# bmorris3/gadfly

Measured on AMD Instinct MI355X. Metric: GP log-likelihood evals/sec (N=1e6, J=30), higher is better.
Workload: dtype f64

## Files before the change

### gadfly_amd/_lib.py

```python
import ctypes
import os
import subprocess

_HERE = os.path.dirname(os.path.abspath(__file__))
CSRC = os.path.join(_HERE, "csrc")
SO_PATH = os.path.join(CSRC, "libgadfly_hip.so")
if os.environ.get("GADFLY_SO"):
    SO_PATH = os.path.abspath(os.environ["GADFLY_SO"])
SOURCES = [os.path.join(CSRC, "gadfly_hip.hip"), os.path.join(CSRC, "gadfly_stored.hip"),
           os.path.join(CSRC, "gadfly_linear.hip"), os.path.join(CSRC, "gadfly_series.hip"),
           os.path.join(CSRC, "gadfly_dense.hip"),
           os.path.join(CSRC, "gadfly_ls.hip"), os.path.join(CSRC, "gadfly_grad.hip"),
           os.path.join(CSRC, "gadfly_solve.hip"), os.path.join(CSRC, "gadfly_predict.hip"),
           os.path.join(CSRC, "gadfly_var.hip"), os.path.join(CSRC, "gadfly_spectral.hip"),
           os.path.join(CSRC, "gadfly_fisher.hip"), os.path.join(CSRC, "gadfly_rhs.hip"),
           os.path.join(CSRC, "gadfly_lsfft.hip"), os.path.join(CSRC, "gadfly_gradtp.hip"),
           os.path.join(CSRC, "gadfly_detrend.hip"), os.path.join(CSRC, "gadfly_linmodel.hip"),
           os.path.join(CSRC, "gadfly_quadform.hip"), os.path.join(CSRC, "gadfly_gradw.hip")]
HEADER = os.path.join(os.path.dirname(_HERE), "include", "gadfly_hip.h")

GF_SOLVE_LOWER, GF_SOLVE_UPPER, GF_MATMUL_LOWER = 0, 1, 2
GF_SWEEP_AUTO, GF_SWEEP_COLUMN, GF_SWEEP_TILED = 0, 1, 2
GF_SWEEP_ZERO_START = 0x100
GF_SWEEP_LONG_SPAN = 0x200
GF_SWEEP_AXIS_PROVEN = 0x400
GF_MAX_WIDTH = 256
GF_GRAD_MAX_WIDTH = 63
GF_GRAD_WORKSPACE_BYTES = 16 << 30
GF_SOLVE_MAX_WIDTH = 63
GF_SOLVE_WORKSPACE_BYTES = 16 << 30
GF_DETREND_MAX_ORDER = 8
GF_LINEAR_MAX_COLS = 255

_lib = None

_vp = ctypes.c_void_p
_i64 = ctypes.c_int64
_int = ctypes.c_int
_dbl = ctypes.c_double

SIGNATURES = {
    "gf_version": (_int, []),
    "gf_last_error": (ctypes.c_char_p, []),
    "gf_leading_dim": (_int, [_int]),
    "gf_build_matrices": (_int, [_int, _i64, _i64, _int, _int, _int] + [_vp] * 7
                          + [_vp, _i64, _vp, _i64] + [_vp] * 4 + [_vp]),
    "gf_state_size": (_i64, [_int]),
    "gf_state_cols": (_int, [_int]),
    "gf_factor": (_int, [_int, _i64, _i64, _int, _int] + [_vp] * 4 + [_vp, _i64]
                  + [_vp] * 6 + [_vp]),
    "gf_scaled_supported": (_int, [_int]),
    "gf_scaled_span": (_dbl, [_int]),
    "gf_scaled_wide_supported": (_int, [_int]),
    "gf_build_scaled": (_int, [_int, _i64, _i64, _int, _int, _int] + [_vp] * 8 + [_int]
                        + [_vp, _i64, _vp, _i64] + [_vp] * 4 + [_vp]),
    "gf_factor_scaled": (_int, [_int, _i64, _i64, _int, _int] + [_vp] * 5 + [_vp, _i64]
                         + [_vp] * 5 + [_vp]),
    "gf_fused_supported": (_int, [_int, _int]),
    "gf_fused_state_size": (_i64, [_int, _int]),
    "gf_loglike_fused": (_int, [_int, _i64, _i64, _int, _int, _int, _int, _int] + [_vp] * 8
                         + [_vp, _i64, _vp, _i64, _vp, _i64] + [_vp] * 5 + [_vp]),
    "gf_steady_size": (_i64, []),
    "gf_loglike_steady": (_int, [_int, _i64, _i64, _int, _int, _int, _int, _int] + [_vp] * 8
                          + [_vp, _i64, _vp, _i64, _vp, _i64] + [_vp] * 5 + [_vp, _i64] + [_vp]),
    "gf_steady_sweep": (_int, [_int, _i64, _i64, _int, _int, _int, _int, _int] + [_vp] * 8
                        + [_vp, _i64, _vp, _i64, _vp, _i64] + [_vp] * 5 + [_vp, _i64] + [_vp]),
    "gf_reduce_tile_steady": (_int, [_int, _i64, _i64] + [_vp] * 5 + [_int, _vp]),
    "gf_steady_sweep_reduced": (_int, [_int, _i64, _i64, _int, _int, _int, _int, _int] + [_vp] * 8
                                + [_vp, _i64, _vp, _i64, _vp, _i64] + [_vp] * 5 + [_vp, _i64, _vp, _int] + [_vp]),
    "gf_steady_sweep_rank1": (_int, [_int, _i64, _i64, _int, _int, _int, _int, _int] + [_vp] * 8
                              + [_vp, _i64, _vp, _i64, _vp, _i64] + [_vp] * 5 + [_vp, _i64, _vp, _int, _vp] + [_vp]),
    "gf_steady_finish": (_int, [_int, _i64, _int, _int, _int, _int] + [_vp] * 5 + [_vp, _i64, _vp, _i64]
                         + [_vp] * 3 + [_vp]),
    "gf_steady_finish_window": (_int, [_int, _i64, _int, _int, _int, _int] + [_vp] * 5 + [_vp, _i64, _vp, _i64]
                                + [_vp] * 3 + [_i64, _i64] + [_vp]),
    "gf_steady_chunk_size": (_i64, [_i64, _int]),
    "gf_steady_finish_chunked": (_int, [_int, _i64, _int, _int, _int, _int] + [_vp] * 5 + [_vp, _i64, _vp, _i64]
                                 + [_vp] * 3 + [_i64, _i64, _int, _vp] + [_vp]),
    "gf_sample_fused": (_int, [_int, _i64, _i64, _int, _int, _int, _int, _int] + [_vp] * 8
                        + [_vp, _i64, _vp, _i64, _vp, _i64] + [_vp] * 5 + [_vp]),
    "gf_chunk_sweep": (_int, [_int, _i64, _i64, _int, _int, _int, _int, _int, _int, _int, _int] + [_vp] * 8
                       + [_vp, _i64, _vp, _i64, _vp, _i64] + [_vp] * 9 + [_vp]),
    "gf_fused_row_stride": (_int, [_int, _int]),
    "gf_scaled_propagator": (_int, [_int, _i64, _int, _int, _vp, _vp, _vp, _vp]),
    "gf_chunk_linear": (_int, [_int, _int, _i64, _i64, _int, _int, _int, _int, _int]
                        + [_vp] * 8 + [_vp]),
    "gf_chunk_linear_combine": (_int, [_int, _int, _i64, _i64, _int, _int, _int] + [_vp] * 5
                                + [_vp]),
    "gf_dense_solve": (_int, [_int, _int, _int] + [_vp] * 2 + [_vp]),
    "gf_dense_solve_logdet": (_int, [_int, _int, _int] + [_vp] * 3 + [_vp]),
    "gf_dense_width": (_int, [_int]),
    "gf_wide_combine_work": (_i64, [_int, _int, _int]),
    "gf_wide_combine": (_int, [_int, _i64, _i64, _int, _int] + [_vp] * 7 + [_vp]),
    "gf_chunk_corrections_work": (_i64, [_int, _int]),
    "gf_chunk_corrections": (_int, [_int, _int, _int, _int, _int] + [_vp] * 6 + [_vp]),
    "gf_wide_gram": (_int, [_int, _i64, _i64, _int, _int, _int, _int, _int] + [_vp] * 5 + [_vp]),
    "gf_lft_tree_work": (_i64, [_int, _int, _int]),
    "gf_lft_tree_scan": (_int, [_int, _int, _int] + [_vp] * 8 + [_vp]),
    "gf_bgemm": (_int, [_int, _int, _int, _int, _int, _int, _vp, _int, _i64, _vp, _int, _i64,
                        _vp, _int, _i64, _vp, _int, _i64, _vp]),
    "gf_chunk_segment_transitions": (_int, [_int, _int, _int] + [_vp] * 4 + [_vp]),
    "gf_chunk_linear_combine_seg": (_int, [_int, _int, _int, _int, _int] + [_vp] * 6 + [_vp]),
    "gf_chunk_transition": (_int, [_int, _i64, _i64, _int, _int, _int, _int, _int, _int] + [_vp] * 9 + [_vp]),
    "gf_chunk_transition_wide": (_int, [_int, _i64, _i64, _int, _int, _int, _int] + [_vp] * 7 + [_vp]),
    "gf_chunk_combine": (_int, [_int, _int, _int] + [_vp] * 5 + [_vp]),
    "gf_chunk_combine_tree_work": (_i64, [_int, _int, _int]),
    "gf_chunk_combine_tree": (_int, [_int, _int, _int, _int] + [_vp] * 8 + [_vp]),
    "gf_reduce_work": (_i64, [_i64]),
    "gf_reduce_tile": (_int, [_int, _i64] + [_vp] * 4 + [_int, _vp]),
    "gf_loglike_finish": (_int, [_int, _i64] + [_vp] * 4 + [_vp]),
    "gf_solve": (_int, [_int, _int, _i64, _int, _int, _int] + [_vp] * 6 + [_vp]),
    "gf_solve_chunk": (_int, [_int, _int, _i64, _i64, _int, _int, _int] + [_vp] * 7 + [_int, _vp]),
    "gf_solve_chunk_rhs": (_int, [_int, _int, _i64, _i64, _int, _int, _int, _int] + [_vp] * 7 + [_int, _vp]),
    "gf_chunk_diag_scan": (_int, [_int, _int, _int, _int, _vp, _vp, _vp]),
    "gf_cross_covariance": (_int, [_int, _i64, _int, _int, _int] + [_vp] * 6 + [_vp, _i64, _vp, _i64, _vp, _vp]),
    "gf_interp_work": (_i64, [_i64]),
    "gf_interp_plan": (_int, [_i64, _vp, _vp, _dbl, _vp, _vp, _vp]),
    "gf_interp_fill": (_int, [_i64, _vp, _vp, _vp, _dbl, _vp, _vp, _vp, _vp]),
    "gf_psd_power": (_int, [_int, _i64, _i64, _dbl, _vp, _vp, _vp]),
    "gf_psd_bin": (_int, [_int, _i64, _int, _vp, _vp, _vp, _dbl, _vp, _vp, _vp]),
    "gf_ls_segments": (_int, [_i64]),
    "gf_ls_work": (_i64, [_i64, _i64, _int]),
    "gf_ls_power": (_int, [_int, _i64, _i64, _i64, _int, _int] + [_vp] * 8 + [_vp]),
    "gf_lsfft_grid": (_i64, [_i64]),
# ... 168 lines not shown
```

### gadfly_amd/csrc/gadfly_hip.hip

```cpp

#include <hip/hip_runtime.h>
#include <atomic>
#include <utility>
#include <type_traits>
#include <stdint.h>
#include <stdio.h>
#include <stdarg.h>
#include <math.h>

#include "../../include/gadfly_hip.h"
#include "gf_internal.h"

#define FM_INLINE __device__ __forceinline__
#include "fastmath.h"
#include "gf_wave.h"
#include "gf_sweep.h"

template <unsigned long long BITS>
__device__ __forceinline__ double fm_local_constant(const int z) {
    return __hiloint2double((int)(unsigned)(BITS >> 32) ^ z, (int)(unsigned)(BITS & 0xffffffffull) ^ z);
}
#define GF_K(x) fm_local_constant<__builtin_bit_cast(unsigned long long, (double)(x))>(fm_z)
__device__ __forceinline__ double fm_exp_local(const double x) {
    int fm_z;
// ... 1231 lines not shown
        for (int j = 0; j < 16; ++j) a[j] = 0.0;
#pragma unroll 4
        for (int k = 0; k < 64; ++k) {
            const double m = s_m[i][k];
#pragma unroll
            for (int j = 0; j < 16; ++j) a[j] = fma(m, s_m[k][c0 + j], a[j]);
        }
    }
#pragma unroll
    for (int j = 0; j < 16; ++j) P[64 * i + c0 + j] = a[j];
}

__global__ void __launch_bounds__(64)
k_steady_chunk_sum(const int B, const int64_t N, const int32_t *__restrict__ info, const double *__restrict__ steady_,
                   const int64_t sw_lo, const int64_t sw_hi, const int64_t chunk_rows,
                   const double *__restrict__ ws_, const int64_t ws_ld, double *__restrict__ acc_) {
    const int pr = blockIdx.x * 64 + threadIdx.x;
    if (pr >= B) return;
    const int64_t sw = steady_chunk_problem(pr, N, info, steady_, sw_lo, sw_hi, chunk_rows, 1);
    if (sw == 0) return;
    const int nch = (int)((N - sw + chunk_rows - 1) / chunk_rows);
    const double *__restrict__ slot = ws_ + (size_t)pr * ws_ld + CH_P;
    double q = 0.0;
    for (int c = 0; c < nch; ++c) q += slot[c * CH_SLOT + 64];
    const double dinf = steady_[(size_t)pr * ST_SIZE + ST_D];
    double *__restrict__ a = acc_ + (size_t)pr * RED_NACC;
    a[0] += (double)(N - sw) * log(dinf);
    a[1] += q / dinf;
    a[2] = fmin(a[2], dinf);
}

constexpr int R1_RR = 0, R1_RI = 64, R1_YR = 128, R1_YI = 192, R1_XR = 256, R1_XI = 320;
constexpr int R1_D = 384, R1_SG = 385;

__device__ __forceinline__ void half_wave_sums(double v, double &lo, double &up) {
    v += dpp_get<0xB1, 0xf>(v);
    v += dpp_get<0x4E, 0xf>(v);
    v += dpp_get<0x141, 0xf>(v);
    v += dpp_get<0x140, 0xf>(v);
    v += dpp_get<0x142, 0xf>(v);
    lo = read_lane(v, 31);
    up = read_lane(v, 63);
}

__device__ __forceinline__ double lane_select(const unsigned long long lanes, const double v, const double keep) {
    int lo = __double2loint(keep), hi = __double2hiint(keep);
    asm("v_cndmask_b32 %0, %0, %1, %2" : "+v"(lo) : "v"(__double2loint(v)), "s"(lanes));
    asm("v_cndmask_b32 %0, %0, %1, %2" : "+v"(hi) : "v"(__double2hiint(v)), "s"(lanes));
    return __hiloint2double(hi, lo);
}

constexpr int R1_UNROLL = 8;

__global__ void __launch_bounds__(64, 2)
k_steady_rank1(const int64_t N, const int64_t n_first, const int Jc, const double gap,
               const double *__restrict__ ac_, const double *__restrict__ bc_,
               const double *__restrict__ cc_, const double *__restrict__ dc_,
               const double *__restrict__ diag_add_, const double *__restrict__ cmax_,
               const double *__restrict__ t_, const int64_t t_bs,
               const double *__restrict__ diag_, const int64_t diag_bs,
               const double *__restrict__ y_, const int64_t y_bs,
               double *__restrict__ d_, double *__restrict__ z_, double *__restrict__ S_state,
               int32_t *__restrict__ info, double *__restrict__ steady_, const int64_t arm_from,
               const double *__restrict__ dt_, double *acc_, const int acc_init) {
    const int lane = threadIdx.x, pr = blockIdx.x;
    const int h = lane >> 5, c = lane & 31;
    int64_t tile_lim = 0;
#define R1_EXIT(lim) do { if (acc_) { tile_lim = (lim); goto tile_sums; } return; } while (0)
  {
    if (info[pr] != 0) R1_EXIT(steady_rows_stored(steady_, pr, N, n_first));
    double *__restrict__ hdr = steady_ + (size_t)pr * ST_SIZE;
    if (hdr[ST_SW] > 0.0) R1_EXIT(steady_rows_stored(steady_, pr, N, n_first));
    const double *__restrict__ tg = t_ + (size_t)pr * t_bs + n_first;
    const double *__restrict__ yg = y_ + (size_t)pr * y_bs + n_first;
    double *__restrict__ dg = d_ + (size_t)pr * N;
    double *__restrict__ zg = z_ + (size_t)pr * N;
    double *__restrict__ Sg = S_state + (size_t)pr * (64 * 64);
    const bool term = c < Jc, fl = lane == 63;
    const size_t ck = (size_t)pr * Jc + (term ? c : 0);
    const double ck_c = term ? cc_[ck] : 0.0, ck_d = term ? dc_[ck] : 0.0;
    const double ck_a = term ? ac_[ck] : 0.0, ck_b = term ? bc_[ck] : 0.0;
    const double wmax = wave_max(fmax(ck_c, fabs(ck_d)));
    const double gthr = gap / cmax_[pr], jthr = 2e-6 / wmax;
    const double delta = dt_[pr];
    double lr, li;
    {
        double sn, cs;
        fm_sincos(ck_d * delta, &sn, &cs);
        const double e = fm_exp(-ck_c * delta);
        lr = e * cs;
        li = -e * sn;
    }
    double rr, ri, Yr, Yi, Xr, Xi, d, sg;
    if (n_first == 0) {
        d = (diag_ ? diag_[(size_t)pr * diag_bs] : 0.0) + diag_add_[pr];
        sg = fast_rcp(d);
        rr = term ? 1.0 : 0.0;
        ri = 0.0;
        Yr = term ? lr : 0.0;
        Yi = term ? li : 0.0;
        Xr = h ? Yr : 0.0;
        Xi = h ? Yi : 0.0;
    } else {
        rr = Sg[R1_RR + lane]; ri = Sg[R1_RI + lane];
        Yr = Sg[R1_YR + lane]; Yi = Sg[R1_YI + lane];
        Xr = Sg[R1_XR + lane]; Xi = Sg[R1_XI + lane];
        d = Sg[R1_D]; sg = Sg[R1_SG];
    }
    constexpr double thr = ST_THR;
    int cnt = __builtin_amdgcn_readfirstlane((int)hdr[ST_CNT]);
    int fill = __builtin_amdgcn_readfirstlane((int)hdr[ST_FILL]);
    int32_t fail = 0;
    double inv = fast_rcp(d);
    double kr = rr * inv, ki = ri * inv;
    const int64_t last = N - 1;
    auto row_of = [&](const int64_t cb) { const int64_t i = cb + lane; return i < last ? i : last; };
    double t_nx, tp_nx, y_nx;
    {
        const int64_t i = row_of(0);
        t_nx = tg[i];
        tp_nx = (n_first + i > 0) ? tg[i - 1] : t_nx - delta;
        y_nx = yg[i];
    }
    double sd = 0.0, sz = 0.0, sr, si, beta, yv_blk = 0.0;
    auto row_front = [&](const int j) __attribute__((always_inline)) {
        const double yy = read_lane(yv_blk, j);
        double sf;
        half_wave_sums(fma(ck_a, Xr, -(ck_b * Xi)), sf, beta);
        const double zn = yy - sf;
// ... 39 lines not shown
        return bad ? (int)__ffsll((long long)bad) - 1 : -1;
    };
    auto flush = [&](const int64_t nb, const int rows) __attribute__((always_inline)) {
        if (lane < rows) { dg[nb + lane] = sd; zg[nb + lane] = sz; }
    };
    const int g0lo = (int)(n_first & (ST_GRID - 1));
    const int ja = (ST_GRID - g0lo) & (ST_GRID - 1);
    __builtin_amdgcn_s_setprio(GF_CHAIN_PRIO);
    for (int64_t nb = 0; nb < N; nb += 64) {
        const int lim = (int)(N - nb < 64 ? N - nb : 64);
        yv_blk = y_nx;
        asm volatile("" : "+v"(yv_blk));
        {
            const double dt = t_nx - tp_nx;
            const bool bad = (dt > gthr) || !(fabs(dt - delta) < jthr);
            if (__any(bad) && lane == 0) hdr[ST_VIOL] = 1.0;
            const int64_t i = row_of(nb + 64);
            t_nx = tg[i];
            tp_nx = (n_first + i > 0) ? tg[i - 1] : t_nx - delta;
            y_nx = yg[i];
        }
        int jf;
        if (ja < lim) {
            plain_rows(0, ja);
            row_front(ja);
            jf = first_failed(ja + 1);
            if (jf < 0) {
                const int64_t n = nb + ja, gn = n_first + n;
                if (gn >= arm_from) {
                    const double x = fl ? d : (h ? ki : kr);
                    double *__restrict__ slot = hdr + ST_RING + (size_t)((gn / ST_GRID) & (ST_LAG - 1)) * 64 + lane;
                    const double xo = *slot;
                    *slot = x;
                    const double dx = fl ? 0.0 : fabs(x - xo);
                    const double mdx = wave_max(dx), mx = wave_max(fl ? 0.0 : fabs(x));
                    const double dold = read_lane(xo, 63);
                    const bool ok = fill >= ST_LAG && mdx <= thr * mx && fabs(d - dold) <= thr * d;
                    cnt = ok ? cnt + 1 : 0;
                    fill = fill < ST_LAG ? fill + 1 : fill;
                    if (lane == 0) { hdr[ST_CNT] = (double)cnt; hdr[ST_FILL] = (double)fill; }
                    if (cnt >= ST_COUNT && gn >= ST_DLAG) {
                        if (h == 0) {
                            hdr[ST_GR + c] = kr;
                            hdr[ST_GI + c] = ki;
                            hdr[ST_SR + c] = sr;
                            hdr[ST_SI + c] = si;
                        }
                        if (lane == 0) {
                            hdr[ST_SW] = (double)(gn + 1);
                            hdr[ST_D] = d;
                            hdr[ST_DT] = (tg[n] - tg[n - ST_DLAG]) * (1.0 / ST_DLAG);
                        }
                        flush(nb, ja + 1);
                        R1_EXIT(n + 1);
                    }
                }
                row_back();
                plain_rows(ja + 1, lim);
                jf = first_failed(lim);
            }
        } else {
            plain_rows(0, lim);
            jf = first_failed(lim);
        }
        if (jf >= 0) {
            flush(nb, jf);
            const int64_t gf = n_first + nb + jf + 1;
            fail = (int32_t)(gf > 0x7fffffff ? 0x7fffffff : gf);
            break;
        }
        flush(nb, lim);
    }
    if (fail) {
        if (lane == 0) info[pr] = fail;
        R1_EXIT(N);
    }
    Sg[R1_RR + lane] = rr; Sg[R1_RI + lane] = ri;
    Sg[R1_YR + lane] = Yr; Sg[R1_YI + lane] = Yi;
    Sg[R1_XR + lane] = Xr; Sg[R1_XI + lane] = Xi;
    if (lane == 0) { Sg[R1_D] = d; Sg[R1_SG] = sg; }
    R1_EXIT(N);
  }
#undef R1_EXIT
tile_sums:
    __builtin_amdgcn_s_setprio(0);
    __builtin_amdgcn_fence(__ATOMIC_RELEASE, "workgroup");
    __builtin_amdgcn_fence(__ATOMIC_ACQUIRE, "workgroup");
    steady_tile_sums(d_ + (size_t)pr * N, z_ + (size_t)pr * N, N, tile_lim, acc_ + (size_t)pr * RED_NACC, acc_init, lane);
}

struct PhiRing {
    static constexpr int PD = 8;
    static constexpr int USL = 72, RSL = 64;
    static constexpr int OD = 64, OE = 66, OZ = 68;
    double u[PD][USL];
    double r[PD + 1][RSL];
};

struct PhiCursor {
    uintptr_t cu, cr, mask;
    unsigned long long ustep;
    bool in_u, in_r;
    unsigned lds_u, lds_r;
    template <int rows = 64>
    __device__ __forceinline__ void init(PhiRing &R, const int lane, const size_t pb, const double *ut_,
                                         const double *rbar_, const double *dbar_, const double *de_,
                                         const double *zbar_) {
        cu = reinterpret_cast<uintptr_t>(ut_ + pb * 64 + 2 * (lane & 31));
        cr = reinterpret_cast<uintptr_t>(rbar_ + pb * 64 + 2 * (lane & 31));
        mask = ~(uintptr_t)0;
        ustep = 64 * 8;
        if (lane >= 32) {
            const double *sp = (lane == 32) ? dbar_ : (lane == 33) ? de_ : zbar_;
            cu = reinterpret_cast<uintptr_t>(sp + pb);
            mask = ~(uintptr_t)15;
            ustep = 8;
        }
        in_u = lane < (rows + 1) / 2 || (lane >= 32 && lane < 35);
        in_r = lane < (rows + 1) / 2;
        lds_u = __builtin_amdgcn_readfirstlane((unsigned)reinterpret_cast<uintptr_t>(&R.u[0][0]));
        lds_r = __builtin_amdgcn_readfirstlane((unsigned)reinterpret_cast<uintptr_t>(&R.r[0][0]));
    }
    __device__ __forceinline__ void issue(const int64_t m, const int after) {
        const unsigned sl = (unsigned)(m & (PhiRing::PD - 1));
        if (in_u) glds16(reinterpret_cast<const void *>(cu & mask), lds_u + sl * (PhiRing::USL * 8), after);
        if (in_r) glds16(reinterpret_cast<const void *>(cr), lds_r + sl * (PhiRing::RSL * 8), after);
        cu += ustep;
        cr += 64 * 8;
    }
};

template <int NT>
struct PhiGram {
    static constexpr int LD = 80;
    static constexpr int NACC = NT * (NT + 1) / 2;
    double hs[16][LD];
    double sv[16];
};

template <int NT>
__device__ __forceinline__ void phi_gram_flush(PhiGram<NT> &Gm, d4 (&acc)[PhiGram<NT>::NACC], const int lane) {
// ... 1443 lines not shown
                                   info, stream));
}

int64_t gf_steady_size(void) { return ST_SIZE; }

int gf_loglike_steady(int B, int64_t N, int64_t n_first, int Jr, int Jc, int block,
                      int gen_period, int variant,
                      const double *ar, const double *cr, const double *ac,
                      const double *bc, const double *cc, const double *dc,
                      const double *diag_add, const double *cmax,
                      const double *t, int64_t t_bs, const double *diag, int64_t diag_bs,
                      const double *y, int64_t y_bs,
                      double *d, double *z, double *S_state, double *F_state,
                      int32_t *info, double *steady, int64_t arm_from, void *stream) {
    if (!steady) return gf_internal_error(-1, "gf_loglike_steady: null pointer");
    SweepCall c = sweep_call("gf_loglike_steady", B, N, n_first, Jr, Jc, block, gen_period, variant, ar, cr, ac, bc, cc, dc,
                             diag_add, cmax, t, t_bs, diag, diag_bs, y, y_bs, d, z, S_state, F_state, info, stream);
    c.steady = steady; c.arm_from = arm_from;
    return launch_sweep(c);
}

int gf_steady_sweep(int B, int64_t N, int64_t n_first, int Jr, int Jc, int block,
                    int gen_period, int variant,
                    const double *ar, const double *cr, const double *ac,
                    const double *bc, const double *cc, const double *dc,
                    const double *diag_add, const double *cmax,
                    const double *t, int64_t t_bs, const double *diag, int64_t diag_bs,
                    const double *y, int64_t y_bs,
                    double *d, double *z, double *S_state, double *F_state,
                    int32_t *info, double *steady, int64_t arm_from, void *stream) {
    if (!steady) return gf_internal_error(-1, "gf_steady_sweep: null pointer");
    SweepCall c = sweep_call("gf_steady_sweep", B, N, n_first, Jr, Jc, block, gen_period, variant, ar, cr, ac, bc, cc, dc,
                             diag_add, cmax, t, t_bs, diag, diag_bs, y, y_bs, d, z, S_state, F_state, info, stream);
    c.steady = steady; c.arm_from = arm_from; c.tail = false;
    return launch_sweep(c);
}

int gf_steady_sweep_reduced(int B, int64_t N, int64_t n_first, int Jr, int Jc, int block,
                            int gen_period, int variant,
                            const double *ar, const double *cr, const double *ac,
                            const double *bc, const double *cc, const double *dc,
                            const double *diag_add, const double *cmax,
                            const double *t, int64_t t_bs, const double *diag, int64_t diag_bs,
                            const double *y, int64_t y_bs,
                            double *d, double *z, double *S_state, double *F_state,
                            int32_t *info, double *steady, int64_t arm_from, double *acc, int init, void *stream) {
    if (!steady || !acc) return gf_internal_error(-1, "gf_steady_sweep_reduced: null pointer");
    SweepCall c = sweep_call("gf_steady_sweep_reduced", B, N, n_first, Jr, Jc, block, gen_period, variant, ar, cr, ac, bc,
                             cc, dc, diag_add, cmax, t, t_bs, diag, diag_bs, y, y_bs, d, z, S_state, F_state, info, stream);
    c.steady = steady; c.arm_from = arm_from; c.tail = false; c.acc = acc; c.acc_init = init ? 1 : 0;
    return launch_sweep(c);
}

int gf_steady_sweep_rank1(int B, int64_t N, int64_t n_first, int Jr, int Jc, int block,
                          int gen_period, int variant,
                          const double *ar, const double *cr, const double *ac,
                          const double *bc, const double *cc, const double *dc,
                          const double *diag_add, const double *cmax,
                          const double *t, int64_t t_bs, const double *diag, int64_t diag_bs,
                          const double *y, int64_t y_bs,
                          double *d, double *z, double *S_state, double *F_state,
                          int32_t *info, double *steady, int64_t arm_from, double *acc, int init,
                          const double *dt, void *stream) {
    const SweepCall c = sweep_call("gf_steady_sweep_rank1", B, N, n_first, Jr, Jc, block, gen_period, variant, ar, cr, ac,
                                   bc, cc, dc, diag_add, cmax, t, t_bs, diag, diag_bs, y, y_bs, d, z, S_state, F_state,
                                   info, stream);
    const char *who = c.who;
    if (B < 1 || N < 1) return gf_internal_error(-1, "%s: empty problem (N=%lld)", who, (long long)N);
    if (check_block(who, block) || check_n_first(who, n_first, block)) return -1;
    if (!t || !y || !d || !z || !S_state || !info || !diag_add || !cmax || !ac || !bc || !cc || !dc || !steady || !dt)
        return gf_internal_error(-1, "%s: null pointer", who);
    if (check_sweep_options(who, gen_period, variant & ~(GF_SWEEP_ZERO_START | GF_SWEEP_LONG_SPAN), Jr, Jc)) return -1;
    if ((variant & GF_SWEEP_ZERO_START) || !sweep_tiled(variant & ~GF_SWEEP_LONG_SPAN, Jr, Jc) || Jc < 1 || arm_from < 0)
        return gf_internal_error(-1, "%s: steady mode is for the streamed lane-tiled sweep only (Jr = 0, Jc <= 31; Jc=%d)", who, Jc);
    hipLaunchKernelGGL(k_steady_rank1, dim3(c.B), dim3(64), 0, c.st, c.N, c.n_first, c.Jc, sweep_gap(block, variant),
                       c.ac, c.bc, c.cc, c.dc, c.diag_add, c.cmax, c.t, c.t_bs, c.diag, c.diag_bs, c.y, c.y_bs, c.d, c.z,
                       c.S_state, c.info, steady, arm_from, dt, acc, init ? 1 : 0);
    return check_launch(who);
}

static int check_finish(const char *who, int B, int64_t N, int Jr, int Jc, int block) {
    if (B < 1 || N < 1) return gf_internal_error(-1, "%s: empty problem (B=%d, N=%lld)", who, B, (long long)N);
    if (Jr != 0 || Jc < 1 || Jc > 31)
        return gf_internal_error(-1, "%s: steady mode is for the lane-tiled sweep only (Jr = 0, Jc <= 31; Jr=%d, Jc=%d)", who, Jr, Jc);
    return check_block(who, block);
}
static int check_window(const char *who, int64_t sw_lo, int64_t sw_hi) {
    if (sw_lo < 0 || sw_hi < sw_lo)
        return gf_internal_error(-1, "%s: the window of switch rows needs 0 <= sw_lo <= sw_hi (sw_lo=%lld, sw_hi=%lld)", who,
                                 (long long)sw_lo, (long long)sw_hi);
    return 0;
}

static int steady_finish_launch(const char *who, int B, int64_t N, int Jr, int Jc, int block, int variant,
                                const double *ac, const double *bc, const double *cc, const double *dc,
                                const double *cmax, const double *t, int64_t t_bs, const double *y, int64_t y_bs,
                                const int32_t *info, double *steady, double *acc, int64_t sw_lo, int64_t sw_hi,
                                void *stream) {
    if (check_finish(who, B, N, Jr, Jc, block)) return -1;
    if (!ac || !bc || !cc || !dc || !cmax || !t || !y || !info || !steady || !acc)
        return gf_internal_error(-1, "%s: null pointer", who);
    if (check_window(who, sw_lo, sw_hi)) return -1;
    if (sw_lo == sw_hi) return 0;
    const double gap = sweep_gap(block, variant & ~GF_SWEEP_AXIS_PROVEN);
    const bool proven = (variant & GF_SWEEP_AXIS_PROVEN) != 0;
    if (!dispatch_rows((2 * Jc + 3) / 4 * 4, [&](auto r) {
            constexpr int R = decltype(r)::value;
            hipLaunchKernelGGL((proven ? k_steady_finish<R, true> : k_steady_finish<R, false>), dim3(B), dim3(64), 0,
                               (hipStream_t)stream, N, Jc, gap, ac, bc, cc, dc, cmax, t, t_bs, y, y_bs, info, steady, acc,
                               sw_lo, sw_hi);
        }))
        return gf_internal_error(-1, "%s: internal dispatch error", who);
    return check_launch(who);
}

int gf_steady_finish(int B, int64_t N, int Jr, int Jc, int block, int variant,
                     const double *ac, const double *bc, const double *cc, const double *dc, const double *cmax,
                     const double *t, int64_t t_bs, const double *y, int64_t y_bs,
                     const int32_t *info, double *steady, double *acc, void *stream) {
    return steady_finish_launch("gf_steady_finish", B, N, Jr, Jc, block, variant, ac, bc, cc, dc, cmax, t, t_bs, y, y_bs,
                                info, steady, acc, 0, INT64_MAX, stream);
}

int gf_steady_finish_window(int B, int64_t N, int Jr, int Jc, int block, int variant,
                            const double *ac, const double *bc, const double *cc, const double *dc, const double *cmax,
                            const double *t, int64_t t_bs, const double *y, int64_t y_bs,
                            const int32_t *info, double *steady, double *acc,
                            int64_t sw_lo, int64_t sw_hi, void *stream) {
    return steady_finish_launch("gf_steady_finish_window", B, N, Jr, Jc, block, variant, ac, bc, cc, dc, cmax, t, t_bs,
                                y, y_bs, info, steady, acc, sw_lo, sw_hi, stream);
// ... 251 lines not shown
```

### gadfly_amd/engine.py

```python
import contextlib
import functools
import math
import typing

import numpy as np

from . import _lib


def _on_device(method):
    @functools.wraps(method)
    def wrapper(self, *args, **kwargs):
        with self.torch.cuda.device(self.device):
            return method(self, *args, **kwargs)
    return wrapper


@functools.lru_cache(maxsize=None)
def _scaled_span(long_span):
    return float(_lib.load().gf_scaled_span(1 if long_span else 0))


def _coeff_pack(coeffs_list):
    Jr = len(coeffs_list[0][0])
# ... 763 lines not shown
        def padded(x):
            buf = torch.zeros((x.shape[0] * x.shape[1] + 4,), **f64)
            buf[:x.numel()] = x.reshape(-1)
            return buf[:x.numel()].view(x.shape[0], x.shape[1]), buf

        t = rows(t, "t")
        self.N = int(t.shape[1])
        self._tmax = float(t.abs().max()) if axis_stats is None else float(axis_stats[0])
        self.t, self._tpad = padded(t)
        y = rows(y, "y")
        if y.shape[1] != self.N:
            raise ValueError("dimension mismatch")
        self.y, self._ypad = padded(y)
        self.diag = None
        if diag is not None:
            diag = rows(diag, "diag")
            if diag.shape[1] != self.N:
                raise ValueError("dimension mismatch")
            self.diag, self._dpad = padded(diag)
        self._diag_amax = None if self.diag is None else self.diag.amax(dim=1)
        self._coeff_host = (real, comp, diag_add, c)
        self._coeffs_list = list(coeffs_list)
        B, ld = self.B, self.ld
        self.scaled = bool(self.lib.gf_scaled_supported(self.W)) and not force_v1
        self.scaled_wide = bool(self.lib.gf_scaled_wide_supported(self.W)) and not force_v1
        self.allow_fused = bool(allow_fused) and self.scaled and self.W <= 63
        self.allow_wide = (bool(allow_fused) and not force_v1 and self.W > 63
                           and bool(self.lib.gf_fused_supported(self.Jr, self.Jc)))
        self.sweep_variant = _lib.GF_SWEEP_AUTO
        self.generator_period = 4
        self.two_sweep = False
        self.steady_state = True
        self.steady_used = False
        self._steady = None
        self._steady_axis = None
        self._steady_cad_max = None
        self._steady_scanned = None
        self.steady_axis_proven = True
        self._steady_from = 0
        self._steady_skip = 0
        self._steady_feedback = None
        self.finish_events = []
        self.steady_overlap = True
        self._steady_split = 0
        self._steady_mid = 0
        self._steady_chunk_blocks = None
        self._steady_chunk_ws = None
        self._steady_mid_ws = None
        self._finish_side = None
        self._finish_mid_side = None
        self._simds = None
        self.steady_sweep_reduces = True
        self.steady_rank1 = True
        self.rank1_used = False
        self._rank1_dt = None
        self._rank1_cond = None
        T = int(min(max(int(tile_rows), 1), self.N))
        if T < self.N:
            T = max(64, T // 64 * 64)
        self.tile_rows = T
        tt = self.t[0]
        if axis_stats is not None:
            self._dt_med = float(axis_stats[1])
        else:
            self._dt_med = float(torch.median(tt[1:] - tt[:-1])) if self.N > 1 else 0.0
        self.axis_stats = (self._tmax, self._dt_med)
        self._pack = self._make_pack(*self._coeff_host)
        self.generator_period = self.period_for_condition(self.NOMINAL_COND) if self.generator_period > 1 else 1
        self.generator_period = min(self.generator_period, 4)

        def rows_buf():
            return torch.zeros((B * T + 2, ld), **f64)

        self._rows_buf = rows_buf
        self._nbuf = 2 if (T < self.N and overlap_build) else 1
        self.bufs = None
        self.d = torch.empty((B, T), **f64)
        self.z = torch.empty((B, T), **f64)
        nS = 64 * 64 if self.scaled else int(self.lib.gf_state_size(self.W))
        if self.allow_wide:
            nS = max(nS, int(self.lib.gf_fused_state_size(self.Jr, self.Jc)))
        nF = 64 if self.scaled else int(self.lib.gf_state_cols(self.W))
        self.S_state = torch.empty((B, nS), **f64)
        self.F_state = torch.empty((B, nF), **f64)
        self.acc = torch.empty((B, 3), **f64)
        self.work = torch.empty((B * int(self.lib.gf_reduce_work(T)),), **f64)
        self.info = torch.zeros((B,), dtype=torch.int32, device=self.device)
        self.out = torch.empty((B,), **f64)
        self.overlap_build = bool(overlap_build)
        self.side = torch.cuda.Stream(device=self.device) if self.overlap_build else None
        self.time_factor = False
        self.factor_events = []

    _bs = staticmethod(_bs)

    def _alloc_bufs(self):
        torch = self.torch
        f64 = dict(dtype=torch.float64, device=self.device)
        n = self.B * self.tile_rows + 2
        self.bufs = [dict(a=torch.zeros((n,), **f64), U=self._rows_buf(), V=self._rows_buf(),
                          P=None if (self.scaled or self.scaled_wide) else self._rows_buf(),
                          de=torch.zeros((n,), **f64))
                     for _ in range(self._nbuf)]

    def _fused_ok(self):
        return self.allow_fused and self._pack.dmax * self._tmax < SINCOS_RANGE
# ... 185 lines not shown
        T, N, B = self.tile_rows, self.N, self.B
        pack = self._pack
        block, variant = sweep_options(pack, self.sweep_variant)
        per_tile = sweep_head(pack, B, 0, 0, self.Jr, self.Jc, block, int(self.generator_period), variant, self.t,
                              self.diag, self.y, self.d, self.z, self.S_state, self.F_state, self.info)[3:]
        self.kernel_used = "fused-wide" if self.W > 63 else "fused"
        arm_from = self._steady_arm_from()
        start = None if arm_from is None else self._steady_plan(arm_from)
        self.rank1_used = arm_from is not None and self._rank1_ok(arm_from)
        if self.rank1_used:
            start = 0
            if self._rank1_dt is None:
                span = (self.t[:, -1] - self.t[:, 0]) / float(max(N - 1, 1))
                self._rank1_dt = span.expand(B).contiguous()
        self.steady_used = start is not None
        if self.steady_used:
            if self._steady is None:
                self._steady = torch.empty((B, int(lib.gf_steady_size())), dtype=torch.float64, device=self.device)
            self._steady.zero_()
        ntiles = (N + T - 1) // T
        overlap = self.steady_used and self.steady_overlap and B >= self.STEADY_OVERLAP_MIN_B
        split = self._steady_split if overlap else 0
        k_e = split // T - 1 if 0 < split < N else -1
        if not 0 <= k_e < ntiles - 1:
            split, k_e = 0, -1
        mid_end = self._steady_mid if split and B >= self.STEADY_MIDDLE_MIN_B else 0
        k_m = mid_end // T - 1 if mid_end % T == 0 else -1
        if not k_e < k_m < ntiles - 1:
            mid_end, k_m = 0, -1
        windows = steady_windows(split, mid_end)
        used = []
        finish_variant = self._finish_variant(pack, block, variant) if self.steady_used else variant

        def side_stream(middle):
            which = "_finish_mid_side" if middle else "_finish_side"
            if getattr(self, which) is None:
                setattr(self, which, torch.cuda.Stream(device=self.device))
            if getattr(self, which) not in used:
                used.append(getattr(self, which))
            return getattr(self, which)

        def chunked(stream, window, cb, which):
            cb = self._steady_chunk_blocks or cb
            ws = getattr(self, which)
            if ws is None or ws[1] != cb:
                ws = (torch.empty((B, int(lib.gf_steady_chunk_size(N, cb))), dtype=torch.float64, device=self.device), cb)
                setattr(self, which, ws)
            finish("gf_steady_finish_chunked", stream, window[0], window[1], cb, p(ws[0]))

        def finish(name, stream, *tail):
            with _timed(torch, self.time_factor, stream, self.finish_events):
                self._finish_launch(name, stream, pack, block, finish_variant, *tail)

        for k in range(ntiles):
            n0 = k * T
            rows = min(T, N - n0)
            args = (B, rows, n0) + per_tile
            steady_tile = self.steady_used and n0 + rows > start
            reduced = steady_tile and split and k > k_e and self.steady_sweep_reduces
            with _timed(torch, self.time_factor, main, self.factor_events, rows):
                if self.rank1_used:
                    st = lib.gf_steady_sweep_rank1(*args, p(self._steady), 0, p(self.acc) if reduced else None,
                                                   1 if k == 0 else 0, p(self._rank1_dt), main.cuda_stream)
                    _lib.check(st, "gf_steady_sweep_rank1")
                elif reduced:
                    st = lib.gf_steady_sweep_reduced(*args, p(self._steady), arm_from, p(self.acc), 1 if k == 0 else 0,
                                                     main.cuda_stream)
                    _lib.check(st, "gf_steady_sweep_reduced")
                elif steady_tile:
                    st = lib.gf_steady_sweep(*args, p(self._steady), arm_from, main.cuda_stream)
                    _lib.check(st, "gf_steady_sweep")
                else:
                    st = lib.gf_loglike_fused(*args, main.cuda_stream)
                    _lib.check(st, "gf_loglike_fused")
            if reduced:
                pass
            elif steady_tile:
                st = lib.gf_reduce_tile_steady(B, rows, n0, p(self.d), p(self.z), p(self._steady), p(self.work),
                                               p(self.acc), 1 if k == 0 else 0, main.cuda_stream)
                _lib.check(st, "gf_reduce_tile_steady")
            else:
                st = lib.gf_reduce_tile(B, rows, p(self.d), p(self.z), p(self.work), p(self.acc),
                                        1 if k == 0 else 0, main.cuda_stream)
                _lib.check(st, "gf_reduce_tile")
            if k == k_e or k == k_m:
                side = side_stream(k == k_m and self.steady_middle_stream)
                side.wait_event(main.record_event())
                if k == k_e:
                    finish("gf_steady_finish_window", side, *windows[0])
                else:
                    chunked(side, windows[1], steady_chunk_blocks(N, 8), "_steady_mid_ws")
        if self.steady_used:
            if split:
                if mid_end:
                    if self._simds is None:
                        self._simds = 4 * torch.cuda.get_device_properties(self.device).multi_processor_count
                    cb = steady_final_chunk_blocks(N, B, self._simds)
                else:
                    cb = steady_chunk_blocks(N, 8)
                chunked(main, windows[-1], cb, "_steady_chunk_ws")
                for side in used:
                    main.wait_stream(side)
            else:
                finish("gf_steady_finish", main)
            sw = self._steady[:, 0]
            swi = torch.where(sw > 0.0, sw, torch.full_like(sw, float("inf")))
            fb = torch.stack([swi.min(), torch.kthvalue(swi, B - B // 8).values,
                              torch.kthvalue(swi, B - B // 64).values, sw.max(), self._rank1_conditions().max()])
            host = torch.zeros((5,), dtype=torch.float64, pin_memory=True)
            host.copy_(torch.where(torch.isfinite(fb), fb, torch.zeros_like(fb)), non_blocking=True)
            done = torch.cuda.Event()
            done.record(main)
            self._steady_feedback = (host, done)
        out = torch.empty((B,), dtype=torch.float64, device=self.device)
        st = lib.gf_loglike_finish(B, N, p(self.acc), p(self.info), p(out), None,
                                   main.cuda_stream)
        _lib.check(st, "gf_loglike_finish")
        return out

    STEADY_PROBE = 16
    STEADY_OVERLAP_MIN_B = 64
    STEADY_MIDDLE_MIN_B = 512
    steady_middle_stream = True

    def _steady_plan(self, arm_from):
        fb = self._steady_feedback
        if fb is not None and fb[1].query():
            (first, most, mid, latest), self._steady_feedback = (int(v) for v in fb[0][:4]), None
            if len(fb[0]) > 4:
                self._rank1_cond = float(fb[0][4])
            if first > 0:
                self._steady_from = max(0, first - self.STEADY_MIN_ROWS - self.tile_rows)
                self._steady_skip = 0
            else:
                self._steady_from, self._steady_skip = 0, self.STEADY_PROBE - 1
            self._steady_split, self._steady_mid = steady_boundaries(self.N, self.tile_rows, most, mid, latest)
        if self._steady_skip > 0:
            self._steady_skip -= 1
            return None
        return max(arm_from, self._steady_from)

    RANK1_JITTER = 1e-7
    RANK1_COND_LIMIT = 1e5
    RANK1_MIN_ROWS = 32768
# ... 495 lines not shown
```

### include/gadfly_hip.h

```cpp
#ifndef GADFLY_HIP_H
#define GADFLY_HIP_H

#include <stdint.h>

#ifdef __cplusplus
extern "C" {
#endif

#define GF_MAX_WIDTH 256

#define GF_SOLVE_LOWER   0
#define GF_SOLVE_UPPER   1
#define GF_MATMUL_LOWER  2

#define GF_SWEEP_AUTO    0
#define GF_SWEEP_COLUMN  1
#define GF_SWEEP_TILED   2
#define GF_SWEEP_ZERO_START 0x100
#define GF_SWEEP_LONG_SPAN 0x200
#define GF_SWEEP_AXIS_PROVEN 0x400

int gf_version(void);
const char *gf_last_error(void);

// ... 34 lines not shown
int gf_fused_supported(int Jr, int Jc);
int64_t gf_fused_state_size(int Jr, int Jc);
int gf_loglike_fused(int B, int64_t N, int64_t n_first, int Jr, int Jc, int block,
                     int gen_period, int variant,
                     const double *ar, const double *cr, const double *ac,
                     const double *bc, const double *cc, const double *dc,
                     const double *diag_add, const double *cmax,
                     const double *t, int64_t t_bs, const double *diag, int64_t diag_bs,
                     const double *y, int64_t y_bs,
                     double *d, double *z, double *S_state, double *F_state,
                     int32_t *info, void *stream);

int64_t gf_steady_size(void);
int gf_loglike_steady(int B, int64_t N, int64_t n_first, int Jr, int Jc, int block,
                      int gen_period, int variant,
                      const double *ar, const double *cr, const double *ac,
                      const double *bc, const double *cc, const double *dc,
                      const double *diag_add, const double *cmax,
                      const double *t, int64_t t_bs, const double *diag, int64_t diag_bs,
                      const double *y, int64_t y_bs,
                      double *d, double *z, double *S_state, double *F_state,
                      int32_t *info, double *steady, int64_t arm_from, void *stream);

int gf_steady_sweep(int B, int64_t N, int64_t n_first, int Jr, int Jc, int block,
                    int gen_period, int variant,
                    const double *ar, const double *cr, const double *ac,
                    const double *bc, const double *cc, const double *dc,
                    const double *diag_add, const double *cmax,
                    const double *t, int64_t t_bs, const double *diag, int64_t diag_bs,
                    const double *y, int64_t y_bs,
                    double *d, double *z, double *S_state, double *F_state,
                    int32_t *info, double *steady, int64_t arm_from, void *stream);
int gf_reduce_tile_steady(int B, int64_t N, int64_t n_first, const double *d, const double *z,
                          const double *steady, double *work, double *acc, int init, void *stream);
int gf_steady_sweep_reduced(int B, int64_t N, int64_t n_first, int Jr, int Jc, int block,
                            int gen_period, int variant,
                            const double *ar, const double *cr, const double *ac,
                            const double *bc, const double *cc, const double *dc,
                            const double *diag_add, const double *cmax,
                            const double *t, int64_t t_bs, const double *diag, int64_t diag_bs,
                            const double *y, int64_t y_bs,
                            double *d, double *z, double *S_state, double *F_state,
                            int32_t *info, double *steady, int64_t arm_from, double *acc, int init, void *stream);
int gf_steady_sweep_rank1(int B, int64_t N, int64_t n_first, int Jr, int Jc, int block,
                          int gen_period, int variant,
                          const double *ar, const double *cr, const double *ac,
                          const double *bc, const double *cc, const double *dc,
                          const double *diag_add, const double *cmax,
                          const double *t, int64_t t_bs, const double *diag, int64_t diag_bs,
                          const double *y, int64_t y_bs,
                          double *d, double *z, double *S_state, double *F_state,
                          int32_t *info, double *steady, int64_t arm_from, double *acc, int init,
                          const double *dt, void *stream);
int gf_steady_finish(int B, int64_t N, int Jr, int Jc, int block, int variant,
                     const double *ac, const double *bc, const double *cc, const double *dc, const double *cmax,
                     const double *t, int64_t t_bs, const double *y, int64_t y_bs,
                     const int32_t *info, double *steady, double *acc, void *stream);
int gf_steady_finish_window(int B, int64_t N, int Jr, int Jc, int block, int variant,
                            const double *ac, const double *bc, const double *cc, const double *dc, const double *cmax,
                            const double *t, int64_t t_bs, const double *y, int64_t y_bs,
                            const int32_t *info, double *steady, double *acc,
                            int64_t sw_lo, int64_t sw_hi, void *stream);
int64_t gf_steady_chunk_size(int64_t N, int chunk_blocks);
int gf_steady_finish_chunked(int B, int64_t N, int Jr, int Jc, int block, int variant,
                             const double *ac, const double *bc, const double *cc, const double *dc, const double *cmax,
                             const double *t, int64_t t_bs, const double *y, int64_t y_bs,
                             const int32_t *info, double *steady, double *acc,
                             int64_t sw_lo, int64_t sw_hi, int chunk_blocks, double *chunk_ws, void *stream);

int gf_sample_fused(int B, int64_t N, int64_t n_first, int Jr, int Jc, int block,
                    int gen_period, int variant,
                    const double *ar, const double *cr, const double *ac,
                    const double *bc, const double *cc, const double *dc,
                    const double *diag_add, const double *cmax,
                    const double *t, int64_t t_bs, const double *diag, int64_t diag_bs,
                    const double *eps, int64_t eps_bs,
                    double *d, double *out, double *S_state, double *F_state,
                    int32_t *info, void *stream);

int gf_chunk_sweep(int B, int64_t N, int64_t chunk_len, int nch, int chunk_first, int chunk_count,
                   int Jr, int Jc, int block, int gen_period, int variant,
                   const double *ar, const double *cr, const double *ac,
                   const double *bc, const double *cc, const double *dc,
                   const double *diag_add, const double *cmax,
                   const double *t, int64_t t_bs, const double *diag, int64_t diag_bs,
                   const double *y, int64_t y_bs,
                   double *d, double *z, double *r_out, double *Ut_out, double *Wt_out,
                   double *de_out, double *S_state, double *F_state,
                   int32_t *info, void *stream);
int gf_chunk_transition(int B, int64_t N, int64_t chunk_len, int nch, int chunk_first, int chunk_count,
                        int Jr, int Jc, int variant, const double *c, const double *de, const double *dbar,
                        const double *zbar, const double *rbar, const double *Ut,
                        double *Phi_out, double *G_out, double *m_out, void *stream);
int gf_fused_row_stride(int Jr, int Jc);
int gf_scaled_propagator(int B, int64_t N, int W, int ld, const double *c, const double *de,
                         double *P_out, void *stream);
int gf_chunk_transition_wide(int B, int64_t N, int64_t chunk_len, int nch, int chunk_first, int chunk_count, int Jc,
                             const double *c, const double *de, const double *dbar, const double *rbar,
                             const double *Ut, double *h_out, double *Phi_out, void *stream);
int gf_chunk_combine(int B, int nch, int W, const double *Phi, const double *G, const double *m,
                     double *S_state, double *F_state, void *stream);
int64_t gf_chunk_combine_tree_work(int B, int P, int nch);
int gf_chunk_combine_tree(int B, int P, int nch, int W, double *Phi, double *G, double *m, double *S, double *F,
                          double *Xst, double *Yst, double *work, void *stream);

int gf_chunk_linear(int mode, int B, int64_t N, int64_t chunk_len, int nch, int W, int R,
// ... 242 lines not shown
```

Measured before the change: 55900.

## Fuse consecutive rank-1 steady tiles into one persistent span kernel launch

Adds a span kernel that loops over several consecutive row tiles inside a single launch, reusing the rank-1 steady sweep body (now a templated device function) with a fixed tile stride. The engine replaces per-tile launches between the finish-window points with one or two span launches, so per-tile launch overhead and host-side per-tile work go away. The trade-off is less interleaving between tiles and the side-stream finish work, plus a higher launch-bounds occupancy hint that may change register allocation.

Measured after the change: 55350. Within noise of the previous version (-1.0%).

```diff
diff --git a/gadfly_amd/_lib.py b/gadfly_amd/_lib.py
--- a/gadfly_amd/_lib.py
+++ b/gadfly_amd/_lib.py
@@ -70,6 +70,9 @@
                                 + [_vp, _i64, _vp, _i64, _vp, _i64] + [_vp] * 5 + [_vp, _i64, _vp, _int] + [_vp]),
     "gf_steady_sweep_rank1": (_int, [_int, _i64, _i64, _int, _int, _int, _int, _int] + [_vp] * 8
                               + [_vp, _i64, _vp, _i64, _vp, _i64] + [_vp] * 5 + [_vp, _i64, _vp, _int, _vp] + [_vp]),
+    "gf_steady_sweep_rank1_span": (_int, [_int, _i64, _i64, _int, _int, _int, _int, _int] + [_vp] * 8
+                                   + [_vp, _i64, _vp, _i64, _vp, _i64] + [_vp] * 5 + [_vp, _i64, _vp, _int, _vp]
+                                   + [_i64, _int] + [_vp]),
     "gf_steady_finish": (_int, [_int, _i64, _int, _int, _int, _int] + [_vp] * 5 + [_vp, _i64, _vp, _i64]
                          + [_vp] * 3 + [_vp]),
     "gf_steady_finish_window": (_int, [_int, _i64, _int, _int, _int, _int] + [_vp] * 5 + [_vp, _i64, _vp, _i64]
diff --git a/gadfly_amd/csrc/gadfly_hip.hip b/gadfly_amd/csrc/gadfly_hip.hip
--- a/gadfly_amd/csrc/gadfly_hip.hip
+++ b/gadfly_amd/csrc/gadfly_hip.hip
@@ -1307,29 +1307,32 @@
 
 constexpr int R1_UNROLL = 8;
 
-__global__ void __launch_bounds__(64, 2)
-k_steady_rank1(const int64_t N, const int64_t n_first, const int Jc, const double gap,
-               const double *__restrict__ ac_, const double *__restrict__ bc_,
-               const double *__restrict__ cc_, const double *__restrict__ dc_,
-               const double *__restrict__ diag_add_, const double *__restrict__ cmax_,
-               const double *__restrict__ t_, const int64_t t_bs,
-               const double *__restrict__ diag_, const int64_t diag_bs,
-               const double *__restrict__ y_, const int64_t y_bs,
-               double *__restrict__ d_, double *__restrict__ z_, double *__restrict__ S_state,
-               int32_t *__restrict__ info, double *__restrict__ steady_, const int64_t arm_from,
-               const double *__restrict__ dt_, double *acc_, const int acc_init) {
+template <bool SPAN>
+__device__ __forceinline__ bool
+steady_rank1_tile(const int64_t N, const int64_t ld_, const int64_t n_first, const int Jc, const double gap,
+                  const double *__restrict__ ac_, const double *__restrict__ bc_,
+                  const double *__restrict__ cc_, const double *__restrict__ dc_,
+                  const double *__restrict__ diag_add_, const double *__restrict__ cmax_,
+                  const double *__restrict__ t_, const int64_t t_bs,
+                  const double *__restrict__ diag_, const int64_t diag_bs,
+                  const double *__restrict__ y_, const int64_t y_bs,
+                  double *__restrict__ d_, double *__restrict__ z_, double *__restrict__ S_state,
+                  int32_t *__restrict__ info, double *__restrict__ steady_, const int64_t arm_from,
+                  const double *__restrict__ dt_, double *acc_, const int acc_init) {
     const int lane = threadIdx.x, pr = blockIdx.x;
     const int h = lane >> 5, c = lane & 31;
+    const int64_t ld = SPAN ? ld_ : N;
     int64_t tile_lim = 0;
-#define R1_EXIT(lim) do { if (acc_) { tile_lim = (lim); goto tile_sums; } return; } while (0)
+    bool more = false;
+#define R1_EXIT(lim, go) do { if (acc_) { tile_lim = (lim); if (SPAN) more = (go); goto tile_sums; } return SPAN && (go); } while (0)
   {
-    if (info[pr] != 0) R1_EXIT(steady_rows_stored(steady_, pr, N, n_first));
+    if (info[pr] != 0) R1_EXIT(steady_rows_stored(steady_, pr, N, n_first), false);
     double *__restrict__ hdr = steady_ + (size_t)pr * ST_SIZE;
-    if (hdr[ST_SW] > 0.0) R1_EXIT(steady_rows_stored(steady_, pr, N, n_first));
+    if (hdr[ST_SW] > 0.0) R1_EXIT(steady_rows_stored(steady_, pr, N, n_first), false);
     const double *__restrict__ tg = t_ + (size_t)pr * t_bs + n_first;
     const double *__restrict__ yg = y_ + (size_t)pr * y_bs + n_first;
-    double *__restrict__ dg = d_ + (size_t)pr * N;
-    double *__restrict__ zg = z_ + (size_t)pr * N;
+    double *__restrict__ dg = d_ + (size_t)pr * ld;
+    double *__restrict__ zg = z_ + (size_t)pr * ld;
     double *__restrict__ Sg = S_state + (size_t)pr * (64 * 64);
     const bool term = c < Jc, fl = lane == 63;
     const size_t ck = (size_t)pr * Jc + (term ? c : 0);
@@ -1475,7 +1478,7 @@
                             hdr[ST_DT] = (tg[n] - tg[n - ST_DLAG]) * (1.0 / ST_DLAG);
                         }
                         flush(nb, ja + 1);
-                        R1_EXIT(n + 1);
+                        R1_EXIT(n + 1, false);
                     }
                 }
                 row_back();
@@ -1496,20 +1499,60 @@
     }
     if (fail) {
         if (lane == 0) info[pr] = fail;
-        R1_EXIT(N);
+        R1_EXIT(N, false);
     }
     Sg[R1_RR + lane] = rr; Sg[R1_RI + lane] = ri;
     Sg[R1_YR + lane] = Yr; Sg[R1_YI + lane] = Yi;
     Sg[R1_XR + lane] = Xr; Sg[R1_XI + lane] = Xi;
     if (lane == 0) { Sg[R1_D] = d; Sg[R1_SG] = sg; }
-    R1_EXIT(N);
+    R1_EXIT(N, true);
   }
 #undef R1_EXIT
 tile_sums:
     __builtin_amdgcn_s_setprio(0);
     __builtin_amdgcn_fence(__ATOMIC_RELEASE, "workgroup");
     __builtin_amdgcn_fence(__ATOMIC_ACQUIRE, "workgroup");
-    steady_tile_sums(d_ + (size_t)pr * N, z_ + (size_t)pr * N, N, tile_lim, acc_ + (size_t)pr * RED_NACC, acc_init, lane);
+    steady_tile_sums(d_ + (size_t)pr * ld, z_ + (size_t)pr * ld, N, tile_lim, acc_ + (size_t)pr * RED_NACC, acc_init, lane);
+    return SPAN && more;
+}
+
+__global__ void __launch_bounds__(64, 2)
+k_steady_rank1(const int64_t N, const int64_t n_first, const int Jc, const double gap,
+               const double *__restrict__ ac_, const double *__restrict__ bc_,
+               const double *__restrict__ cc_, const double *__restrict__ dc_,
+               const double *__restrict__ diag_add_, const double *__restrict__ cmax_,
+               const double *__restrict__ t_, const int64_t t_bs,
+               const double *__restrict__ diag_, const int64_t diag_bs,
+               const double *__restrict__ y_, const int64_t y_bs,
+               double *__restrict__ d_, double *__restrict__ z_, double *__restrict__ S_state,
+               int32_t *__restrict__ info, double *__restrict__ steady_, const int64_t arm_from,
+               const double *__restrict__ dt_, double *acc_, const int acc_init) {
+    steady_rank1_tile<false>(N, N, n_first, Jc, gap, ac_, bc_, cc_, dc_, diag_add_, cmax_, t_, t_bs, diag_, diag_bs,
+                      y_, y_bs, d_, z_, S_state, info, steady_, arm_from, dt_, acc_, acc_init);
+}
+
+__global__ void __launch_bounds__(64, 4)
+k_steady_rank1_span(const int64_t N, const int64_t n_first, const int64_t tile_rows, const int tiles, const int Jc,
+                    const double gap,
+                    const double *__restrict__ ac_, const double *__restrict__ bc_,
+                    const double *__restrict__ cc_, const double *__restrict__ dc_,
+                    const double *__restrict__ diag_add_, const double *__restrict__ cmax_,
+                    const double *__restrict__ t_, const int64_t t_bs,
+                    const double *__restrict__ diag_, const int64_t diag_bs,
+                    const double *__restrict__ y_, const int64_t y_bs,
+                    double *__restrict__ d_, double *__restrict__ z_, double *__restrict__ S_state,
+                    int32_t *__restrict__ info, double *__restrict__ steady_, const int64_t arm_from,
+                    const double *__restrict__ dt_, double *acc_, const int acc_init) {
+#pragma unroll 1
+    for (int k = 0; k < tiles; ++k) {
+        const int64_t n0 = (int64_t)k * tile_rows;
+        const int64_t rows = N - n0 < tile_rows ? N - n0 : tile_rows;
+        if (rows < 1) return;
+        if (!steady_rank1_tile<true>(rows, tile_rows, n_first + n0, Jc, gap, ac_, bc_, cc_, dc_, diag_add_,
+                                     cmax_, t_, t_bs, diag_, diag_bs, y_, y_bs, d_, z_, S_state, info, steady_, arm_from,
+                                     dt_, acc_, k == 0 ? acc_init : 0))
+            return;
+    }
 }
 
 struct PhiRing {
@@ -3059,6 +3102,20 @@
     return launch_sweep(c);
 }
 
+static int check_rank1(const SweepCall &c, int block, int gen_period, int variant, const double *steady, int64_t arm_from,
+                       const double *dt) {
+    const char *who = c.who;
+    if (c.B < 1 || c.N < 1) return gf_internal_error(-1, "%s: empty problem (N=%lld)", who, (long long)c.N);
+    if (check_block(who, block) || check_n_first(who, c.n_first, block)) return -1;
+    if (!c.t || !c.y || !c.d || !c.z || !c.S_state || !c.info || !c.diag_add || !c.cmax || !c.ac || !c.bc || !c.cc ||
+        !c.dc || !steady || !dt)
+        return gf_internal_error(-1, "%s: null pointer", who);
+    if (check_sweep_options(who, gen_period, variant & ~(GF_SWEEP_ZERO_START | GF_SWEEP_LONG_SPAN), c.Jr, c.Jc)) return -1;
+    if ((variant & GF_SWEEP_ZERO_START) || !sweep_tiled(variant & ~GF_SWEEP_LONG_SPAN, c.Jr, c.Jc) || c.Jc < 1 || arm_from < 0)
+        return gf_internal_error(-1, "%s: steady mode is for the streamed lane-tiled sweep only (Jr = 0, Jc <= 31; Jc=%d)", who, c.Jc);
+    return 0;
+}
+
 int gf_steady_sweep_rank1(int B, int64_t N, int64_t n_first, int Jr, int Jc, int block,
                           int gen_period, int variant,
                           const double *ar, const double *cr, const double *ac,
@@ -3072,17 +3129,40 @@
     const SweepCall c = sweep_call("gf_steady_sweep_rank1", B, N, n_first, Jr, Jc, block, gen_period, variant, ar, cr, ac,
                                    bc, cc, dc, diag_add, cmax, t, t_bs, diag, diag_bs, y, y_bs, d, z, S_state, F_state,
                                    info, stream);
-    const char *who = c.who;
-    if (B < 1 || N < 1) return gf_internal_error(-1, "%s: empty problem (N=%lld)", who, (long long)N);
-    if (check_block(who, block) || check_n_first(who, n_first, block)) return -1;
-    if (!t || !y || !d || !z || !S_state || !info || !diag_add || !cmax || !ac || !bc || !cc || !dc || !steady || !dt)
-        return gf_internal_error(-1, "%s: null pointer", who);
-    if (check_sweep_options(who, gen_period, variant & ~(GF_SWEEP_ZERO_START | GF_SWEEP_LONG_SPAN), Jr, Jc)) return -1;
-    if ((variant & GF_SWEEP_ZERO_START) || !sweep_tiled(variant & ~GF_SWEEP_LONG_SPAN, Jr, Jc) || Jc < 1 || arm_from < 0)
-        return gf_internal_error(-1, "%s: steady mode is for the streamed lane-tiled sweep only (Jr = 0, Jc <= 31; Jc=%d)", who, Jc);
+    if (check_rank1(c, block, gen_period, variant, steady, arm_from, dt)) return -1;
     hipLaunchKernelGGL(k_steady_rank1, dim3(c.B), dim3(64), 0, c.st, c.N, c.n_first, c.Jc, sweep_gap(block, variant),
                        c.ac, c.bc, c.cc, c.dc, c.diag_add, c.cmax, c.t, c.t_bs, c.diag, c.diag_bs, c.y, c.y_bs, c.d, c.z,
                        c.S_state, c.info, steady, arm_from, dt, acc, init ? 1 : 0);
+    return check_launch(c.who);
+}
+
+int gf_steady_sweep_rank1_span(int B, int64_t N, int64_t n_first, int Jr, int Jc, int block,
+                               int gen_period, int variant,
+                               const double *ar, const double *cr, const double *ac,
+                               const double *bc, const double *cc, const double *dc,
+                               const double *diag_add, const double *cmax,
+                               const double *t, int64_t t_bs, const double *diag, int64_t diag_bs,
+                               const double *y, int64_t y_bs,
+                               double *d, double *z, double *S_state, double *F_state,
+                               int32_t *info, double *steady, int64_t arm_from, double *acc, int init,
+                               const double *dt, int64_t tile_rows, int tiles, void *stream) {
+    const SweepCall c = sweep_call("gf_steady_sweep_rank1_span", B, N, n_first, Jr, Jc, block, gen_period, variant, ar, cr,
+                                   ac, bc, cc, dc, diag_add, cmax, t, t_bs, diag, diag_bs, y, y_bs, d, z, S_state, F_state,
+                                   info, stream);
+    const char *who = c.who;
+    if (check_rank1(c, block, gen_period, variant, steady, arm_from, dt)) return -1;
+    if (!acc) return gf_internal_error(-1, "%s: null pointer", who);
+    if (tiles < 1 || tile_rows < 1)
+        return gf_internal_error(-1, "%s: a span needs tiles >= 1 and tile_rows >= 1 (tiles=%d, tile_rows=%lld)", who,
+                                 tiles, (long long)tile_rows);
+    if (N <= (int64_t)(tiles - 1) * tile_rows || N > (int64_t)tiles * tile_rows)
+        return gf_internal_error(-1, "%s: N=%lld rows are not %d tiles of tile_rows=%lld", who, (long long)N, tiles,
+                                 (long long)tile_rows);
+    if (tiles > 1 && tile_rows % block != 0)
+        return gf_internal_error(-1, "%s: tile_rows=%lld must be a multiple of block=%d", who, (long long)tile_rows, block);
+    hipLaunchKernelGGL(k_steady_rank1_span, dim3(c.B), dim3(64), 0, c.st, c.N, c.n_first, tile_rows, tiles, c.Jc,
+                       sweep_gap(block, variant), c.ac, c.bc, c.cc, c.dc, c.diag_add, c.cmax, c.t, c.t_bs, c.diag,
+                       c.diag_bs, c.y, c.y_bs, c.d, c.z, c.S_state, c.info, steady, arm_from, dt, acc, init ? 1 : 0);
     return check_launch(who);
 }
 
diff --git a/gadfly_amd/engine.py b/gadfly_amd/engine.py
--- a/gadfly_amd/engine.py
+++ b/gadfly_amd/engine.py
@@ -839,6 +839,8 @@
         self._simds = None
         self.steady_sweep_reduces = True
         self.steady_rank1 = True
+        self.steady_span = True
+        self.span_events = []
         self.rank1_used = False
         self._rank1_dt = None
         self._rank1_cond = None
@@ -1130,7 +1132,19 @@
             with _timed(torch, self.time_factor, stream, self.finish_events):
                 self._finish_launch(name, stream, pack, block, finish_variant, *tail)
 
-        for k in range(ntiles):
+        def finish_behind(k):
+            side = side_stream(k == k_m and self.steady_middle_stream)
+            side.wait_event(main.record_event())
+            if k == k_e:
+                finish("gf_steady_finish_window", side, *windows[0])
+            else:
+                chunked(side, windows[1], steady_chunk_blocks(N, 8), "_steady_mid_ws")
+
+        spans = []
+        if (self.rank1_used and split and self.steady_span and self.steady_sweep_reduces
+                and getattr(lib, "gf_steady_sweep_rank1_span", None) is not None):
+            spans = [(k_e + 1, k_m), (k_m + 1, ntiles - 1)] if k_m >= 0 else [(k_e + 1, ntiles - 1)]
+        for k in range(spans[0][0] if spans else ntiles):
             n0 = k * T
             rows = min(T, N - n0)
             args = (B, rows, n0) + per_tile
@@ -1162,12 +1176,16 @@
                                         1 if k == 0 else 0, main.cuda_stream)
                 _lib.check(st, "gf_reduce_tile")
             if k == k_e or k == k_m:
-                side = side_stream(k == k_m and self.steady_middle_stream)
-                side.wait_event(main.record_event())
-                if k == k_e:
-                    finish("gf_steady_finish_window", side, *windows[0])
-                else:
-                    chunked(side, windows[1], steady_chunk_blocks(N, 8), "_steady_mid_ws")
+                finish_behind(k)
+        for first, last in spans:
+            n0 = first * T
+            rows = min(N, (last + 1) * T) - n0
+            with _timed(torch, self.time_factor, main, self.span_events, rows):
+                st = lib.gf_steady_sweep_rank1_span(B, rows, n0, *per_tile, p(self._steady), 0, p(self.acc), 0,
+                                                    p(self._rank1_dt), T, last - first + 1, main.cuda_stream)
+                _lib.check(st, "gf_steady_sweep_rank1_span")
+            if last == k_m:
+                finish_behind(last)
         if self.steady_used:
             if split:
                 if mid_end:
diff --git a/include/gadfly_hip.h b/include/gadfly_hip.h
--- a/include/gadfly_hip.h
+++ b/include/gadfly_hip.h
@@ -110,6 +110,16 @@
                           double *d, double *z, double *S_state, double *F_state,
                           int32_t *info, double *steady, int64_t arm_from, double *acc, int init,
                           const double *dt, void *stream);
+int gf_steady_sweep_rank1_span(int B, int64_t N, int64_t n_first, int Jr, int Jc, int block,
+                               int gen_period, int variant,
+                               const double *ar, const double *cr, const double *ac,
+                               const double *bc, const double *cc, const double *dc,
+                               const double *diag_add, const double *cmax,
+                               const double *t, int64_t t_bs, const double *diag, int64_t diag_bs,
+                               const double *y, int64_t y_bs,
+                               double *d, double *z, double *S_state, double *F_state,
+                               int32_t *info, double *steady, int64_t arm_from, double *acc, int init,
+                               const double *dt, int64_t tile_rows, int tiles, void *stream);
 int gf_steady_finish(int B, int64_t N, int Jr, int Jc, int block, int variant,
                      const double *ac, const double *bc, const double *cc, const double *dc, const double *cmax,
                      const double *t, int64_t t_bs, const double *y, int64_t y_bs,
```
